# deeprob-org/deeprob-kit

Measured on AMD Instinct MI355X. Metric: log-likelihoods/sec, RAT-SPN D=784 batch=64k at 1/2/4/8 MI355X, higher is better.
Workload: dtype f32; 1 GPU; GaussianRatSpn(784, rg_depth=2, rg_repetitions=8, rg_batch=2, rg_sum=2) forward LL, 65536 samples per GPU per step, mean LL reduced on device; global_batch=65536, resident_batches=4

## Files before the change

### deeprob-kit_amd/csrc/ratspn_gemm_common.h

```cpp
#pragma once
#include "common.h"
#include <math.h>

namespace dpk {

typedef _Float16 half8 __attribute__((ext_vector_type(8)));
typedef _Float16 half4 __attribute__((ext_vector_type(4)));
typedef _Float16 half2 __attribute__((ext_vector_type(2)));
typedef float gf32x2 __attribute__((ext_vector_type(2)));
typedef float gf32x4 __attribute__((ext_vector_type(4)));
typedef float gf32x16 __attribute__((ext_vector_type(16)));

constexpr int kGemmWaves = 4;
constexpr int kGemmTile = 32 * kGemmWaves;
constexpr int kGemmStages = 3;
#ifndef DPK_X_NT
#define DPK_X_NT 0
#endif
constexpr bool kGemmXNonTemporal = DPK_X_NT != 0;
typedef __attribute__((address_space(3))) float lfloat;
typedef __attribute__((address_space(3))) unsigned lunsigned;
typedef __attribute__((address_space(3))) char lchar;
typedef const __attribute__((address_space(1))) char *gcchar_p;
typedef const __attribute__((address_space(1))) void *gvoid_p;
__host__ __device__ constexpr int gemm_ks(int NT) { return NT <= 2 ? 4 : 2; }
constexpr float kGemmStepBound = 1.0e6f;
constexpr float kGemmAbsBound = 1.0e3f;

__device__ __forceinline__ void split_f16(float v, _Float16 &hi, _Float16 &lo) {
    hi = (_Float16)v;
    lo = (_Float16)(v - (float)hi);
}

__device__ __forceinline__ void gemm_lds_barrier() {
    asm volatile("s_waitcnt lgkmcnt(0)\n\ts_barrier" ::: "memory");
}

template <bool NT = false>
__device__ __forceinline__ void glds16(unsigned voff, gcchar_p sbase_in, unsigned lds_dst_in) {
    const uint64_t sb = (uint64_t)(uintptr_t)sbase_in;
    const uint64_t sbase = ((uint64_t)(unsigned)__builtin_amdgcn_readfirstlane((int)(unsigned)(sb >> 32)) << 32) |
                           (uint64_t)(unsigned)__builtin_amdgcn_readfirstlane((int)(unsigned)sb);
    const unsigned lds_dst = (unsigned)__builtin_amdgcn_readfirstlane((int)lds_dst_in);
    unsigned keep;
    if constexpr (NT)
        asm volatile("s_mov_b32 %0, m0\n\ts_mov_b32 m0, %3\n\ts_nop 4\n\tglobal_load_lds_dwordx4 %1, %2 nt\n\ts_mov_b32 m0, %0"
                     : "=&s"(keep)
                     : "v"(voff), "s"(sbase), "s"(lds_dst)
                     : "memory");
    else
        asm volatile("s_mov_b32 %0, m0\n\ts_mov_b32 m0, %3\n\ts_nop 4\n\tglobal_load_lds_dwordx4 %1, %2\n\ts_mov_b32 m0, %0"
                     : "=&s"(keep)
                     : "v"(voff), "s"(sbase), "s"(lds_dst)
                     : "memory");
}

__device__ __forceinline__ void split8(const float (&v)[8], half8 &xh, half8 &xl) {
#ifdef DPK_SPLIT8_ASM
    typedef unsigned u32x4 __attribute__((ext_vector_type(4)));
    u32x4 hp, lp;
#pragma unroll
    for (int p = 0; p < 4; ++p) {
        unsigned h2, l2;
        float b0, b1;
        asm("v_cvt_pk_f16_f32 %0, %1, %2" : "=v"(h2) : "v"(v[2 * p]), "v"(v[2 * p + 1]));
        asm("v_cvt_f32_f16_e32 %0, %1" : "=v"(b0) : "v"(h2));
        asm("v_cvt_f32_f16_sdwa %0, %1 dst_sel:DWORD dst_unused:UNUSED_PAD src0_sel:WORD_1" : "=v"(b1) : "v"(h2));
        const float d0 = v[2 * p] - b0, d1 = v[2 * p + 1] - b1;
        asm("v_cvt_pk_f16_f32 %0, %1, %2" : "=v"(l2) : "v"(d0), "v"(d1));
        hp[p] = h2;
        lp[p] = l2;
    }
    xh = __builtin_bit_cast(half8, hp);
    xl = __builtin_bit_cast(half8, lp);
    return;
#endif
#pragma unroll
    for (int p = 0; p < 4; ++p) {
        const gf32x2 a = {v[2 * p], v[2 * p + 1]};
        const half2 h = __builtin_convertvector(a, half2);
        const gf32x2 b = __builtin_convertvector(h, gf32x2);
        const half2 l = __builtin_convertvector(a - b, half2);
        xh[2 * p] = h[0];
        xh[2 * p + 1] = h[1];
        xl[2 * p] = l[0];
        xl[2 * p + 1] = l[1];
    }
}


template <int KS, int PB, int PB2 = 0>
__device__ __forceinline__ void gemm_loader_run(const float *x, int64_t B, int D, int NCH, int ntiles, int tile0,
                                                int tstride, gcchar_p table, int chunk_table_bytes, int tab_kb0,
                                                unsigned smem_base, int stage_bytes, int wave, int lane,
                                                gcchar_p table2 = nullptr) {
    constexpr int KC = 16 * KS, W = 4 * KS, ROWB = KC * 4, RPI = 64 / W;
    constexpr int SWS = (W == 16) ? 0 : (W == 8 ? 1 : 2);
    constexpr int XB = kGemmTile * ROWB;
    constexpr int PX = 32 / RPI;
    constexpr int P = PX + PB + PB2;
    static_assert(P <= 63, "vmcnt field");
    unsigned voff[PX];
#pragma unroll
    for (int j = 0; j < PX; ++j) {
        const int rl = wave * 32 + j * RPI + lane / W;
        const int gp = (lane & (W - 1)) ^ ((rl >> SWS) & (W - 1));
        voff[j] = (unsigned)(rl * D + gp * 4) * 4u;
    }
    const unsigned toff = (unsigned)(tab_kb0 * 1024 + lane * 16);
    int ptile = tile0, pc = 0, pstage = 0;
    auto issue_next = [&]() {
        const int64_t b0 = (int64_t)ptile * kGemmTile;
        const gcchar_p xt = (gcchar_p)x + (b0 * D + pc * KC) * 4;
        const gcchar_p tsrc = table + (int64_t)pc * chunk_table_bytes;
        const unsigned st = smem_base + pstage * stage_bytes;
        const bool full = (b0 + kGemmTile <= B) && ((pc + 1) * KC <= D);
        if (full) {
#pragma unroll
            for (int j = 0; j < PX; ++j) glds16<kGemmXNonTemporal>(voff[j], xt, st + (wave * 32 + j * RPI) * ROWB);
        } else {
            const int nvalid = (int)min((int64_t)kGemmTile, B - b0);
            const int vp = min(W, (D - pc * KC) >> 2);
#pragma unroll
            for (int j = 0; j < PX; ++j) {
                const int rl = wave * 32 + j * RPI + lane / W;
                const int gp = min((lane & (W - 1)) ^ ((rl >> SWS) & (W - 1)), vp - 1);
                glds16<kGemmXNonTemporal>((unsigned)(min(rl, nvalid - 1) * D + gp * 4) * 4u, xt, st + (wave * 32 + j * RPI) * ROWB);
            }
        }
#pragma unroll
        for (int j = 0; j < PB; ++j) glds16(toff + j * 1024, tsrc, st + XB + tab_kb0 * 1024 + j * 1024);
        if constexpr (PB2 > 0) {
            const gcchar_p tsrc2 = table2 + (int64_t)pc * chunk_table_bytes;
#pragma unroll
            for (int j = 0; j < PB2; ++j)
                glds16((unsigned)((wave * PB2 + j) * 1024 + lane * 16), tsrc2, st + XB + chunk_table_bytes + (wave * PB2 + j) * 1024);
        }
        pstage = (pstage + 1 == kGemmStages) ? 0 : pstage + 1;
        if (++pc == NCH) {
            pc = 0;
            ptile += tstride;
        }
    };
    static_assert(kGemmStages == 3, "the counted waits leave exactly one chunk in flight");
#pragma unroll
    for (int g = 0; g < kGemmStages - 1; ++g)
        if (ptile < ntiles) issue_next();
    __syncthreads();
    for (int tile = tile0; tile < ntiles; tile += tstride) {
        for (int c = 0; c < NCH; ++c) {
            if (c + 1 < NCH || tile + tstride < ntiles) {
                asm volatile("s_waitcnt vmcnt(%0)" ::"n"(P) : "memory");
            } else {
                asm volatile("s_waitcnt vmcnt(0)" ::: "memory");
            }
            gemm_lds_barrier();
            if (ptile < ntiles) issue_next();
        }
    }
}

}
```

### deeprob-kit_amd/csrc/ratspn_gemm_slice.hip

```cpp
#include "ratspn_gemm_fused.h"
#include "ratspn_gemm_prep.h"
#include "../../include/deeprob_slice.h"
#include <stdlib.h>
#include <algorithm>
#include <atomic>
#include <mutex>
#include <type_traits>
#include <vector>

namespace dpk {

constexpr int kSliceCompute = 7;
constexpr int kSliceKW = 7;
constexpr int kSliceThreads = (kSliceCompute + 1) * 64;
constexpr int kSliceSlot = kSliceKW * 2048;

__host__ __device__ constexpr int slice_part_bytes(int NT) { return NT * 4 * 1024; }
__host__ __device__ constexpr int slice_lds_bytes(int NT, int w0_floats) {
    return kSliceCompute * kSliceSlot + kSliceCompute * slice_part_bytes(NT) + kSliceCompute * 256 + 128 + 1024 + 0 * w0_floats;
}

#ifdef DPK_TIMELINE
#define SL_STAMP(row, slot) do { __builtin_amdgcn_sched_barrier(0); if (a.dbg && lane == 0 && (row) < 16 && blockIdx.x < 256) a.dbg[(((int64_t)blockIdx.x * 8 + wave) * 16 + (row)) * 8 + (slot)] = __builtin_amdgcn_s_memtime(); __builtin_amdgcn_sched_barrier(0); } while (0)
#else
#define SL_STAMP(row, slot) do { } while (0)
#endif

template <int I, int S, int NT>
__device__ __forceinline__ void slice_exact_raw(const GemmArgs &a, const float *raw0, const float *rawr, int64_t bw0, int lane,
                                                LseScratch sc) {
    constexpr int RPT = 8 / I;
    constexpr int RH = (NT * RPT + 1) / 2;
    const int s = lane & 31, h = lane >> 5;
    const int64_t b = bw0 + s;
    const bool valid = b < a.B;
    const float *xr = a.x + (valid ? b : a.B - 1) * a.D;
    const int d = a.d;
    float n1[RH][2][S];
#pragma unroll
    for (int m = 0; m < RH; ++m) {
        const int rho = 2 * m + h;
        float leaf[4][I];
#pragma unroll
        for (int q = 0; q < 4; ++q)
#pragma unroll
            for (int k = 0; k < I; ++k) leaf[q][k] = 0.f;
        if (rho < a.reps) {
#pragma unroll
            for (int q = 0; q < 4; ++q) {
                const int r = rho * 4 + q;
                for (int j = 0; j < d; ++j) {
                    const int64_t o = (int64_t)r * d + j;
                    if (a.pad != nullptr && a.pad[o]) continue;
                    const float xv = xr[a.mask[o]];
#pragma unroll
                    for (int k = 0; k < I; ++k) {
                        const int64_t po = ((int64_t)r * I + k) * d + j;
                        const float mu = a.loc[po], sg = a.scale[po];
                        const float dlt = xv - mu;
                        leaf[q][k] += nan_to_num_f(fmaf(dlt * dlt, -0.5f / (sg * sg), -logf(sg) - kLogSqrt2Pi));
                    }
                }
            }
#pragma unroll
            for (int p = 0; p < 2; ++p)
                prodsum_node_raw<I, S>(leaf[2 * p], leaf[2 * p + 1], raw0 + ((int64_t)rho * 2 + p) * S * I * I, sc.slot, n1[m][p]);
        }
    }
    const int M = a.reps * S * S;
    double part = 0.0;
    for (int cl = 0; cl < a.C; ++cl) {
        const float lse_row = raw_row_lse(rawr + (int64_t)cl * M, M);
        float mm = -INFINITY, ss = 0.f;
#pragma unroll
        for (int m = 0; m < RH; ++m) {
            const int rho = 2 * m + h;
            if (rho < a.reps) {
                float pm, ps;
                root_partial_raw<S>(n1[m][0], n1[m][1], rawr + (int64_t)cl * M + rho * S * S, lse_row, sc.slot, pm, ps);
                lse_merge(mm, ss, pm, ps);
            }
        }
        const float om = __shfl_xor(mm, 32, 64), os = __shfl_xor(ss, 32, 64);
        lse_merge(mm, ss, om, os);
        const float ll = (mm > -INFINITY) ? mm + logf(ss) : -INFINITY;
        if (h == 0 && valid) {
            a.out[b * a.C + cl] = ll;
            part += (double)ll;
        }
    }
    if (a.ll_sum != nullptr) {
        part = wave_reduce_sum(part);
        if (lane == 0) atomicAdd(a.ll_sum, part);
    }
}

constexpr int kSliceShards = 16;
struct SliceVerify {
    unsigned long long verdict[kSliceShards];
    unsigned long long hashed, hashed_base;
    unsigned long long pad[14];
    struct { unsigned long long n, pad[15]; } tickets[kSliceShards];
};
static_assert(sizeof(SliceVerify) == kSliceVerifyBytes, "the workspace block behind the VerifyCtl (common.h)");
__device__ __forceinline__ SliceVerify *slice_verify_of(VerifyCtl *c) {
    return reinterpret_cast<SliceVerify *>(reinterpret_cast<char *>(c) + 64);
}
constexpr int kFpK = 32;
template <int K>
__device__ __forceinline__ void fpw_issue(const unsigned *p, int nwords, int tid, int nthreads, unsigned (&w)[K]) {
#pragma unroll
    for (int k = 0; k < K; ++k) {
        const int e = tid + nthreads * k;
        w[k] = p[e < nwords ? e : 0];
    }
}
template <int K>
__device__ __forceinline__ unsigned long long fpw_sum(const unsigned (&w)[K], int nwords, unsigned tag, int tid, int nthreads) {
    unsigned long long h = 0ull;
#pragma unroll
    for (int k = 0; k < K; ++k) {
        const int e = tid + nthreads * k;
        if (e < nwords) h += fp_word(w[k], (unsigned)e * 8u + tag);
    }
    return h;
}
typedef unsigned fp_u4 __attribute__((ext_vector_type(4)));
template <int K>
__device__ __forceinline__ void fpw_issue4(const unsigned *p, int nwords, int tid, int nthreads, fp_u4 (&w)[K]) {
    const fp_u4 *p4 = (const fp_u4 *)p;
#pragma unroll
    for (int k = 0; k < K; ++k) {
        const int e = tid + nthreads * k;
        w[k] = p4[4 * e < nwords ? e : 0];
    }
}
template <int K>
__device__ __forceinline__ unsigned long long fpw_sum4(const fp_u4 (&w)[K], int nwords, unsigned tag, int tid, int nthreads) {
    unsigned long long h = 0ull;
#pragma unroll
    for (int k = 0; k < K; ++k) {
        const int e = 4 * (tid + nthreads * k);
        if (e < nwords)
            h += (fp_word(w[k].x, (unsigned)e * 8u + tag) + fp_word(w[k].y, (unsigned)(e + 1) * 8u + tag)) +
                 (fp_word(w[k].z, (unsigned)(e + 2) * 8u + tag) + fp_word(w[k].w, (unsigned)(e + 3) * 8u + tag));
    }
    return h;
}
template <int I>
__device__ __forceinline__ unsigned long long slice_hash_share(const GemmPrepArgs &a, int blk, int tid, int nthreads) {
    constexpr int RPT = 8 / I;
    const int nrb = a.NT * RPT, d = a.d;
    if (blk < nrb) {
        if (blk >= a.reps) return 0ull;
        const int rho = blk;
        const int nm = 8 * d, npd = a.pad != nullptr ? d : 0, nl = 4 * I * d;
        const unsigned *pm = (const unsigned *)(a.mask + (int64_t)rho * 4 * d);
        const unsigned *pl = (const unsigned *)(a.loc + (int64_t)rho * 4 * I * d);
        const unsigned *ps = (const unsigned *)(a.scale + (int64_t)rho * 4 * I * d);
        const unsigned *pp = a.pad != nullptr ? (const unsigned *)(a.pad + (int64_t)rho * 4 * d) : pm;
        if (nl > kFpK * nthreads || nm > kFpK * nthreads || npd > 8 * nthreads || ((uintptr_t)pp & 3) != 0 ||
            (((uintptr_t)pm | (uintptr_t)pl | (uintptr_t)ps) & 15) != 0)
            return gemm_prep_hash_share<I>(a, blk, tid, nthreads);
        fp_u4 wm[kFpK / 4], wl[kFpK / 4], ws[kFpK / 4];
        unsigned wp[8];
        fpw_issue4(pm, nm, tid, nthreads, wm);
        fpw_issue4(pl, nl, tid, nthreads, wl);
        fpw_issue4(ps, nl, tid, nthreads, ws);
        fpw_issue(pp, npd > 0 ? npd : 1, tid, nthreads, wp);
        return (fpw_sum4(wm, nm, 1, tid, nthreads) + fpw_sum(wp, npd, 2, tid, nthreads)) +
               (fpw_sum4(wl, nl, 3, tid, nthreads) + fpw_sum4(ws, nl, 4, tid, nthreads));
    }
    constexpr int rpb = kGemmPrepThreads / 64;
    unsigned long long h = 0ull;
    unsigned wv[rpb];
    bool in[rpb];
    unsigned tg[rpb];
#pragma unroll
    for (int r = 0; r < rpb; ++r) {
        const int row = (blk - nrb) * rpb + r;
        int rr = row, m = -1;
#pragma unroll
        for (int mm = 0; mm < 3; ++mm) {
            if (m < 0) {
                if (rr < a.rows[mm]) m = mm;
                else rr -= a.rows[mm];
            }
        }
        const int n = m >= 0 ? a.n[m] : 0;
        if (n > nthreads) return gemm_prep_hash_share<I>(a, blk, tid, nthreads);
        in[r] = tid < n;
        const float *base = m >= 0 ? a.w[m] + (int64_t)rr * n : a.w[0];
        wv[r] = __float_as_uint(base[in[r] ? tid : 0]);
        tg[r] = (unsigned)tid * 8u + (5u + 8192u * (unsigned)row);
    }
#pragma unroll
    for (int r = 0; r < rpb; ++r)
        if (in[r]) h += fp_word(wv[r], tg[r]);
    return h;
}
template <int I>
__device__ __forceinline__ void slice_verify_share(const GemmPrepArgs &pa, int lane, lunsigned *ctl_l) {
    const int np = pa.np, G = (int)gridDim.x, g = (int)blockIdx.x;
    SliceVerify *sv = slice_verify_of(pa.ctl);
    const int shard = g & (kSliceShards - 1);
    if (g >= np) {
        if (lane == 0) {
            const unsigned long long t = __hip_atomic_fetch_add(&sv->tickets[shard].n, 1ull, __ATOMIC_RELAXED, __HIP_MEMORY_SCOPE_AGENT);
            ctl_l[0] = 0u;
            ctl_l[2] = (unsigned)t;
            ctl_l[3] = (unsigned)(t >> 32);
        }
        return;
    }
    const unsigned long long vold = __hip_atomic_load(&sv->verdict[lane & (kSliceShards - 1)], __ATOMIC_RELAXED, __HIP_MEMORY_SCOPE_AGENT);
    const unsigned long long hb = __hip_atomic_load(&sv->hashed_base, __ATOMIC_RELAXED, __HIP_MEMORY_SCOPE_AGENT);
    const unsigned long long stored = pa.hash[g];
    unsigned long long h = slice_hash_share<I>(pa, g, lane, 64);
#pragma unroll
    for (int o = 32; o > 0; o >>= 1) h += (unsigned long long)__shfl_xor((long long)h, o, 64);
    const bool mismatch = kPrepHashBase + (unsigned long long)g + h != stored;
    unsigned long long t = 0ull, r = 0ull;
    if (lane == 0) {
        t = __hip_atomic_fetch_add(&sv->tickets[shard].n, 1ull, __ATOMIC_RELAXED, __HIP_MEMORY_SCOPE_AGENT);
        r = __hip_atomic_fetch_add(&sv->hashed, 1ull + (mismatch ? (1ull << 32) : 0ull), __ATOMIC_RELAXED, __HIP_MEMORY_SCOPE_AGENT);
        ctl_l[0] = 0u;
        ctl_l[2] = (unsigned)t;
        ctl_l[3] = (unsigned)(t >> 32);
    }
    const unsigned rlo = (unsigned)__builtin_amdgcn_readfirstlane((int)(unsigned)r);
    const unsigned rhi = (unsigned)__builtin_amdgcn_readfirstlane((int)(unsigned)(r >> 32));
    const unsigned hblo = (unsigned)__builtin_amdgcn_readfirstlane((int)(unsigned)hb);
    const unsigned hbhi = (unsigned)__builtin_amdgcn_readfirstlane((int)(unsigned)(hb >> 32));
    if (rlo - hblo != (unsigned)(np - 1)) return;
    const unsigned mism_now = rhi + (mismatch ? 1u : 0u);
    const bool stale = mism_now != hbhi;
    if (lane == 0)
        __hip_atomic_store(&sv->hashed_base, ((unsigned long long)mism_now << 32) | (unsigned long long)(rlo + 1u), __ATOMIC_RELAXED,
                           __HIP_MEMORY_SCOPE_AGENT);
    if (lane < kSliceShards) {
        const int cnt = lane < G ? (G - 1 - lane) / kSliceShards + 1 : 0;
        __hip_atomic_store(&sv->verdict[lane], (((vold >> 1) + (unsigned long long)cnt) << 1) | (stale ? 1ull : 0ull), __ATOMIC_RELAXED,
                           __HIP_MEMORY_SCOPE_AGENT);
    }
    if (lane == 0) ctl_l[0] = 2u | (stale ? 1u : 0u);
}
__device__ __forceinline__ void slice_verdict_poll(const GemmPrepArgs &pa, lunsigned *ctl_l, unsigned long long until) {
    const int shard = (int)blockIdx.x & (kSliceShards - 1);
    const unsigned long long *vp = &slice_verify_of(pa.ctl)->verdict[shard];
    const unsigned long long n = ((unsigned long long)ctl_l[3] << 32) | ctl_l[2];
    while ((ctl_l[0] & 2u) == 0u && __builtin_amdgcn_s_memrealtime() < until) {
        const unsigned long long v = __hip_atomic_load(vp, __ATOMIC_RELAXED, __HIP_MEMORY_SCOPE_AGENT);
        if ((v >> 1) > n) ctl_l[0] = 2u | (unsigned)(v & 1ull);
        else __builtin_amdgcn_s_sleep(16);
    }
}
__device__ __forceinline__ void slice_verdict_wait(const GemmPrepArgs &pa, lunsigned *ctl_l) {
    if ((ctl_l[0] & 2u) != 0u) return;
    const int shard = (int)blockIdx.x & (kSliceShards - 1);
    const unsigned long long *vp = &slice_verify_of(pa.ctl)->verdict[shard];
    const unsigned long long n = ((unsigned long long)ctl_l[3] << 32) | ctl_l[2];
    unsigned long long v = __hip_atomic_load(vp, __ATOMIC_RELAXED, __HIP_MEMORY_SCOPE_AGENT);
    bool timed_out = false;
    if ((v >> 1) <= n) {
        const unsigned long long t0 = __builtin_amdgcn_s_memrealtime();
        do {
            __builtin_amdgcn_s_sleep(8);
            v = __hip_atomic_load(vp, __ATOMIC_RELAXED, __HIP_MEMORY_SCOPE_AGENT);
            timed_out = __builtin_amdgcn_s_memrealtime() - t0 > 100000000ull;
        } while ((v >> 1) <= n && !timed_out);
    }
    ctl_l[0] = 2u | ((v & 1ull) != 0ull || timed_out ? 1u : 0u);
}

template <int I, int S, int NT>
__global__ __launch_bounds__(kSliceThreads) void ratspn_gemm_slice_kernel(const GemmArgs a, const GemmPrepArgs pa) {
    constexpr int RPT = 8 / I;
    constexpr int NMAX = (I > S ? I : S);
    constexpr int KW = kSliceKW;
    constexpr int PW = slice_part_bytes(NT);
    constexpr float kL2E = 1.4426950408889634f, kLn2 = 0.6931471805599453f;
    static_assert(I == 2 && NT == 2 && NT * RPT == 8, "phase-2 roles: 8 repetitions x 2 partitions = the 16 lanes of a sample; one b128 per partition");
    typedef __attribute__((address_space(3))) const gf32x4 lf4;
    typedef __attribute__((address_space(3))) gf32x4 lf4w;

    extern __shared__ __attribute__((aligned(16))) char smem_generic[];
    lchar *smem = (lchar *)smem_generic;
    lchar *part_l = smem + kSliceCompute * kSliceSlot;
    lfloat *q_l = (lfloat *)(part_l + kSliceCompute * PW);
    lunsigned *flag_l = (lunsigned *)(q_l + kSliceCompute * 64);
    lunsigned *ctl_l = flag_l + 16;
    lfloat *c2_l = (lfloat *)(flag_l + 32);

    const int tid = threadIdx.x;
    const int lane = tid & 63;
    const int wave = __builtin_amdgcn_readfirstlane(tid >> 6);
    const int s = lane & 31, h = lane >> 5;
    const int D = a.D;
    const int nblk = a.ntiles;
    const int first = (int)blockIdx.x, stride = (int)gridDim.x;
    const bool slicer = wave < kSliceCompute;
    SL_STAMP(15, 0);
    unsigned long long t_poll = 0ull;
    if (!slicer && pa.np > 0) {
        const unsigned long long t_entry = __builtin_amdgcn_s_memrealtime();
        __builtin_amdgcn_s_setprio(3);
        slice_verify_share<I>(pa, lane, ctl_l);
        __builtin_amdgcn_s_setprio(0);
        t_poll = t_entry + (a.ntiles > (int)gridDim.x ? 500ull : 450ull);
    }

    const int k0 = wave * KW;
    lchar *my = smem + (slicer ? wave : 0) * kSliceSlot;
    const unsigned my_u = (unsigned)(uintptr_t)my;
    unsigned voff[2];
#pragma unroll
    for (int i = 0; i < 2; ++i) {
        const int P = i * 64 + lane, drow = P >> 2, dcol = (P & 3) ^ ((drow >> 2) & 3);
        voff[i] = (unsigned)(drow * D + k0 * 16 + dcol * 4) * 4u;
    }
    auto issue_kk = [&](gcchar_p xt, int nvalid, int kk) {
        if (nvalid >= 32) {
            glds16<kGemmXNonTemporal>(voff[0] + kk * 64u, xt, my_u + kk * 2048);
            glds16<kGemmXNonTemporal>(voff[1] + kk * 64u, xt, my_u + kk * 2048 + 1024);
        } else {
#pragma unroll
            for (int i = 0; i < 2; ++i) {
                const int P = i * 64 + lane, drow = P >> 2, dcol = (P & 3) ^ ((drow >> 2) & 3);
                glds16<kGemmXNonTemporal>((unsigned)(min(drow, nvalid - 1) * D + (k0 + kk) * 16 + dcol * 4) * 4u, xt,
                                          my_u + kk * 2048 + i * 1024);
            }
        }
    };
    auto issue = [&](int blk) {
        const int64_t b0 = (int64_t)blk * 32;
        const gcchar_p xt = (gcchar_p)(a.x + b0 * D);
        const int nvalid = (int)min((int64_t)32, a.B - b0);
#pragma unroll
        for (int kk = 0; kk < KW; ++kk) issue_kk(xt, nvalid, kk);
    };
    const int nit = first < nblk ? (nblk - first + stride - 1) / stride : 0;
    lchar *tl = part_l + (slicer ? wave : 0) * PW;
    static_assert(PW >= KW * NT * kSliceTabBytes + 1024, "compact table + keep-masks in the wave's partial block");
    if (slicer && nit > 0) {
        const unsigned tl_u = (unsigned)(uintptr_t)tl;
        glds16<false>((unsigned)lane * 16u, (gcchar_p)pa.smask + wave * 1024, tl_u + KW * NT * kSliceTabBytes);
#pragma unroll
        for (int kk = 0; kk < KW; ++kk)
            glds16<false>((unsigned)lane * 16u, (gcchar_p)pa.stab + (int64_t)(k0 + kk) * NT * kSliceTabBytes,
                          tl_u + kk * NT * kSliceTabBytes);
        issue(first);
    }
    half8 mh[KW][NT], ml[KW][NT];
    typedef unsigned gu32x4 __attribute__((ext_vector_type(4)));
    typedef __attribute__((address_space(3))) const gu32x4 lu4;
    typedef __attribute__((address_space(3))) const unsigned short lushort;
#define DPK_SL_TABLE_EXPAND(kk)                                                                                                \
    do {                                                                                                                      \
        const unsigned bits = *(lushort *)(tl + KW * NT * kSliceTabBytes + lane * 16 + (kk) * 2);                             \
        const lchar *te = tl + (kk) * NT * kSliceTabBytes + ((lane >> 5) * 8 + ((lane >> 3) & 3) * 2 + (lane & 1)) * 16;      \
        _Pragma("unroll") for (int t = 0; t < NT; ++t) {                                                                      \
            gu32x4 hi = *(lu4 *)(te + t * kSliceTabBytes);                                                                    \
            gu32x4 lo = *(lu4 *)(te + t * kSliceTabBytes + kSliceTabBytes / 2);                                               \
            _Pragma("unroll") for (int jj = 0; jj < 4; ++jj) {                                                                \
                const int e0 = __builtin_amdgcn_sbfe((int)bits, t * 8 + 2 * jj, 1);                                           \
                const int e1 = __builtin_amdgcn_sbfe((int)bits, t * 8 + 2 * jj + 1, 1);                                       \
                const unsigned keep = ((unsigned)e0 & 0xFFFFu) | ((unsigned)e1 & 0xFFFF0000u);                                \
                hi[jj] &= keep;                                                                                               \
                lo[jj] &= keep;                                                                                               \
            }                                                                                                                 \
            mh[kk][t] = __builtin_bit_cast(half8, hi);                                                                        \
            ml[kk][t] = __builtin_bit_cast(half8, lo);                                                                        \
        }                                                                                                                     \
    } while (0)
    const int sl = lane >> 4, j = lane & 15;
    const int rho = j >> 1, p = j & 1;
    const int s2 = wave * 4 + sl;
    const bool active = rho < a.reps;
    const int rc = active ? rho : a.reps - 1;
    const int t2 = rc / RPT, ap = rc - t2 * RPT;
    static_assert(S * I * I == 8 && 2 * I == 4 && S * S == 4, "slot record layout");
    if (wave == 7 && sl == 0) {
        const float *wp = a.W0 + ((int64_t)(rc * 2 + p) * S) * I * I;
#pragma unroll
        for (int e = 0; e < S * I * I; ++e) c2_l[j * 16 + e] = wp[e];
#pragma unroll
        for (int qq = 0; qq < 2; ++qq)
#pragma unroll
            for (int k = 0; k < I; ++k) c2_l[j * 16 + 8 + qq * I + k] = a.biasT[(p * NT + t2) * 16 + (ap * 2 + qq) * I + k];
#pragma unroll
        for (int e = 0; e < S * S; ++e) c2_l[j * 16 + 12 + e] = ((const float *)a.Wr)[rc * S * S + e];
    }
    if (!slicer && pa.np > 0 && lane == 0) slice_verdict_poll(pa, ctl_l, t_poll);
    bool model_ok;
    {
        cint_p ce = as_const(a.elig);
        unsigned bits = 0u;
#pragma unroll
        for (int e = 0; e < NT * RPT; ++e) bits |= (ce[e] != 0 ? 1u : 0u) << e;
        model_ok = ((bits >> rc) & 1u) != 0u;
    }
    const int M = a.reps * S * S;
    const float *wr0 = (const float *)a.Wr + rc * S * S;
    if (tid < 16) flag_l[tid] = 0u;

    const int sw = (s >> 2) & 3;
    constexpr int XROW = 64, XKK = 2048;
    const lchar *xr0 = my + s * XROW + (((h * 2) ^ sw) << 4);
    const lchar *xr1 = my + s * XROW + (((h * 2 + 1) ^ sw) << 4);
    lchar *pw = part_l + (slicer ? wave : 0) * PW + s * 256;

    double ll_part = 0.0, pend_part = 0.0;
    bool saw_nan = false;
    unsigned long long exact_mask = 0ull;
    gf32x16 acc[NT];
    float qlane = 0.f;
#define DPK_SL_KSTEP(kk, v, tq2)                                                                                              \
    do {                                                                                                                      \
        _Pragma("unroll") for (int i = 0; i < 8; i += 2) {                                                                    \
            const gf32x2 pv = {v[i], v[i + 1]};                                                                               \
            tq2 = __builtin_elementwise_fma(pv, pv, tq2);                                                                     \
        }                                                                                                                     \
        half8 xh, xl;                                                                                                         \
        split8(v, xh, xl);                                                                                                    \
        _Pragma("unroll") for (int t = 0; t < NT; ++t) acc[t] = __builtin_amdgcn_mfma_f32_32x32x16_f16(mh[kk][t], xh, acc[t], 0, 0, 0); \
        _Pragma("unroll") for (int t = 0; t < NT; ++t) acc[t] = __builtin_amdgcn_mfma_f32_32x32x16_f16(mh[kk][t], xl, acc[t], 0, 0, 0); \
        _Pragma("unroll") for (int t = 0; t < NT; ++t) acc[t] = __builtin_amdgcn_mfma_f32_32x32x16_f16(ml[kk][t], xh, acc[t], 0, 0, 0); \
    } while (0)
    if (slicer && nit > 0) {
        const bool more = nit > 1;
        const int64_t nb0 = (int64_t)(first + stride) * 32;
        const gcchar_p nxt = (gcchar_p)(a.x + nb0 * D);
        const int nnv = (int)min((int64_t)32, a.B - nb0);
#pragma unroll
        for (int t = 0; t < NT; ++t)
#pragma unroll
            for (int i = 0; i < 16; ++i) acc[t][i] = 0.f;
        gf32x2 tq2 = {0.f, 0.f};
        gf32x4 xa0, xa1, xb0, xb1;
        asm volatile("s_waitcnt vmcnt(14)" ::: "memory");
        DPK_SL_TABLE_EXPAND(0);
        asm volatile("s_waitcnt vmcnt(12)" ::: "memory");
        xa0 = *(lf4 *)(xr0);
        xa1 = *(lf4 *)(xr1);
#define DPK_SL_FIRST_STEP(kk, NW_MORE, NW_LAST)                                                                               \
    do {                                                                                                                      \
        asm volatile("s_waitcnt lgkmcnt(0)" ::: "memory");                                                                    \
        if (more && (kk) <= 2) issue_kk(nxt, nnv, kk);                                                                        \
        float v[8];                                                                                                           \
        _Pragma("unroll") for (int i = 0; i < 4; ++i) {                                                                       \
            v[i] = xa0[i];                                                                                                    \
            v[4 + i] = xa1[i];                                                                                                \
        }                                                                                                                     \
        if ((kk) + 1 < KW) {                                                                                                  \
            if (more) asm volatile("s_waitcnt vmcnt(%0)" ::"n"(NW_MORE) : "memory");                                          \
            else asm volatile("s_waitcnt vmcnt(%0)" ::"n"(NW_LAST) : "memory");                                               \
            xb0 = *(lf4 *)(xr0 + ((kk) + 1) * XKK);                                                                           \
            xb1 = *(lf4 *)(xr1 + ((kk) + 1) * XKK);                                                                           \
        }                                                                                                                     \
        if ((kk) + 1 < KW) DPK_SL_TABLE_EXPAND(((kk) + 1 < KW ? (kk) + 1 : 0));                                               \
        DPK_SL_KSTEP(kk, v, tq2);                                                                                             \
        xa0 = xb0;                                                                                                            \
        xa1 = xb1;                                                                                                            \
    } while (0)
        DPK_SL_FIRST_STEP(0, 12, 10);
        DPK_SL_FIRST_STEP(1, 12, 8);
        DPK_SL_FIRST_STEP(2, 12, 6);
        DPK_SL_FIRST_STEP(3, 10, 4);
        DPK_SL_FIRST_STEP(4, 8, 2);
        DPK_SL_FIRST_STEP(5, 6, 0);
        DPK_SL_FIRST_STEP(6, 0, 0);
#undef DPK_SL_FIRST_STEP
#undef DPK_SL_TABLE_EXPAND
        qlane = tq2[0] + tq2[1];
        if (more) {
            issue_kk(nxt, nnv, 3);
            issue_kk(nxt, nnv, 4);
        }
    }
    SL_STAMP(15, 1);
    [[maybe_unused]] int row = 0;
    int it = 0;
    for (; it < nit; ++it) {
        const int blk = first + it * stride;
        const bool more = it + 1 < nit;
        const bool more2 = it + 2 < nit;
        SL_STAMP(row, 0);
        gemm_lds_barrier();
        SL_STAMP(row, 1);
        if (slicer) {
#pragma unroll
            for (int t = 0; t < NT; ++t)
#pragma unroll
                for (int i4 = 0; i4 < 4; ++i4) {
                    const int g = t * 4 + i4;
                    const gf32x4 o = {acc[t][4 * i4], acc[t][4 * i4 + 1], acc[t][4 * i4 + 2], acc[t][4 * i4 + 3]};
                    *(lf4w *)(pw + (((g * 2 + h) ^ (s & 7)) << 4)) = o;
                }
            q_l[wave * 64 + lane] = qlane;
        }
        if (it > 0) {
            const lunsigned *fl = flag_l + ((it - 1) & 1) * 8;
            const unsigned any_bad = (unsigned)__builtin_amdgcn_readfirstlane(
                (int)((fl[0] | fl[1]) | (fl[2] | fl[3]) | (fl[4] | fl[5]) | (fl[6] | fl[7])));
            if (any_bad) exact_mask |= 1ull << (it - 1);
            else ll_part += pend_part;
        }
        gemm_lds_barrier();
        if (slicer && more) {
            const int64_t nb0 = (int64_t)(first + (it + 1) * stride) * 32;
            const gcchar_p nxt = (gcchar_p)(a.x + nb0 * D);
            const int nnv = (int)min((int64_t)32, a.B - nb0);
            issue_kk(nxt, nnv, 5);
            issue_kk(nxt, nnv, 6);
        }
        SL_STAMP(row, 2);

        int jo = j;
        asm volatile("" : "+v"(jo));
        const lchar *pr = part_l + s2 * 256 + ((jo ^ (s2 & 7)) << 4);
        const lfloat *qr = q_l + (jo < 2 * kSliceCompute ? (jo >> 1) * 64 + (jo & 1) * 32 + s2 : 0);
        gf32x4 lf = *(lf4 *)pr;
#pragma unroll
        for (int w = 1; w < kSliceCompute; ++w) lf += *(lf4 *)(pr + w * PW);
        float qv = *qr;
        qv = j < 2 * kSliceCompute ? qv : 0.f;
        const float qtot = row16_sum(qv);
        const int64_t b2 = (int64_t)blk * 32 + s2;
        saw_nan = saw_nan || (qtot != qtot);
        bool bad = !(qtot <= kExpandBound * kExpandBound * (float)D) || (active && !model_ok);
        const lf4 *c2 = (const lf4 *)(c2_l + jo * 16);
        const gf32x4 w0a = c2[0], w0b = c2[1], cs4 = c2[2], wr4 = c2[3];
        const float w0[S][I * I] = {{w0a[0], w0a[1], w0a[2], w0a[3]}, {w0b[0], w0b[1], w0b[2], w0b[3]}};
        float va[I], vc[I];
#pragma unroll
        for (int k = 0; k < I; ++k) {
            va[k] = lf[k] + cs4[k];
            vc[k] = lf[I + k] + cs4[I + k];
        }
        float ea[I], ec[I];
        const float ma = exp2_children<I>(va, ea), mc = exp2_children<I>(vc, ec);
        float n1[S];
#pragma unroll
        for (int o = 0; o < S; ++o) {
            float v = 0.f;
#pragma unroll
            for (int i = 0; i < I; ++i) {
                float tt = 0.f;
#pragma unroll
                for (int jj = 0; jj < I; ++jj) tt = fmaf(w0[o][i * I + jj], ec[jj], tt);
                v = fmaf(ea[i], tt, v);
            }
            n1[o] = fmaf(__builtin_amdgcn_logf(v), kLn2, ma + mc);
            bad = bad || (v < 1e-30f && active);
        }
        float ta[S], tc[S];
#pragma unroll
        for (int o = 0; o < S; ++o) {
            const float other = dpp_f<kDppXor1>(n1[o]);
            ta[o] = p == 0 ? n1[o] : other;
            tc[o] = p == 0 ? other : n1[o];
        }
        float ra[S], rcx[S];
        const float m2 = exp2_children<S>(ta, ra) + exp2_children<S>(tc, rcx);
        const float mr = active ? m2 : -INFINITY;
        const float mtop = row16_max(mr);
        const float mtop0 = (mtop == -INFINITY) ? 0.f : mtop;
        const float scale = (active && p == 0) ? __builtin_amdgcn_exp2f((mr - mtop0) * kL2E) : 0.f;
        const float qterm = -0.5f * qtot;
        const bool writer = j == 0 && b2 < a.B;
        double part = 0.0;
        for (int cl = 0; cl < a.C; ++cl) {
            float wr[S * S];
            if (cl == 0) {
#pragma unroll
                for (int e = 0; e < S * S; ++e) wr[e] = wr4[e];
            } else {
#pragma unroll
                for (int e = 0; e < S * S; ++e) wr[e] = wr0[(int64_t)cl * M + e];
            }
            float v = 0.f;
#pragma unroll
            for (int i = 0; i < S; ++i) {
                float tt = 0.f;
#pragma unroll
                for (int jj = 0; jj < S; ++jj) tt = fmaf(wr[i * S + jj], rcx[jj], tt);
                v = fmaf(ra[i], tt, v);
            }
            bad = bad || (v < 1e-30f && mr > -INFINITY);
            const float tot = row16_sum(v * scale);
            const float ll = ((mtop > -INFINITY) ? fmaf(__builtin_amdgcn_logf(tot), kLn2, mtop) : -INFINITY) + qterm;
            if (writer) {
                a.out[b2 * a.C + cl] = ll;
                part += (double)ll;
            }
        }
        pend_part = part;
        const bool wave_bad = __any(bad);
        if (lane == 0) flag_l[(it & 1) * 8 + wave] = wave_bad ? 1u : 0u;
        SL_STAMP(row, 3);
        if (slicer && more) {
            const int64_t nb2 = (int64_t)(first + (it + 2) * stride) * 32;
            const gcchar_p nxt = (gcchar_p)(a.x + nb2 * D);
            const int nnv = (int)min((int64_t)32, a.B - nb2);
#pragma unroll
            for (int t = 0; t < NT; ++t)
#pragma unroll
                for (int i = 0; i < 16; ++i) acc[t][i] = 0.f;
            gf32x2 tq2 = {0.f, 0.f};
            gf32x4 xa0, xa1, xb0, xb1;
#define DPK_SL_LAND(p)                                                                                                        \
    do {                                                                                                                      \
        if (more2) asm volatile("s_waitcnt vmcnt(%0)" ::"n"(2 * (6 - (p)) + 2 * ((p) < 3 ? (p) : 3)) : "memory");              \
        else asm volatile("s_waitcnt vmcnt(%0)" ::"n"(12 - 2 * (p)) : "memory");                                              \
    } while (0)
            DPK_SL_LAND(0);
            xa0 = *(lf4 *)(xr0);
            xa1 = *(lf4 *)(xr1);
#define DPK_SL_STEP(kk)                                                                                                       \
    do {                                                                                                                      \
                                     \
        asm volatile("s_waitcnt lgkmcnt(0)" ::: "memory");                                                                    \
        if (more2 && (kk) <= 2) issue_kk(nxt, nnv, kk);                                                                       \
        float v[8];                                                                                                           \
        _Pragma("unroll") for (int i = 0; i < 4; ++i) {                                                                       \
            v[i] = xa0[i];                                                                                                    \
            v[4 + i] = xa1[i];                                                                                                \
        }                                                                                                                     \
        if ((kk) + 1 < KW) {                                                                                                  \
            DPK_SL_LAND(((kk) + 1 < KW ? (kk) + 1 : 6));                                                                      \
            xb0 = *(lf4 *)(xr0 + ((kk) + 1) * XKK);                                                                           \
            xb1 = *(lf4 *)(xr1 + ((kk) + 1) * XKK);                                                                           \
        }                                                                                                                     \
        DPK_SL_KSTEP(kk, v, tq2);                                                                                             \
        xa0 = xb0;                                                                                                            \
        xa1 = xb1;                                                                                                            \
    } while (0)
            DPK_SL_STEP(0);
            DPK_SL_STEP(1);
            DPK_SL_STEP(2);
            DPK_SL_STEP(3);
            DPK_SL_STEP(4);
            DPK_SL_STEP(5);
            DPK_SL_STEP(6);
#undef DPK_SL_STEP
#undef DPK_SL_LAND
            qlane = tq2[0] + tq2[1];
            if (more2) {
                issue_kk(nxt, nnv, 3);
                issue_kk(nxt, nnv, 4);
            }
        }
        SL_STAMP(row, 4);
        ++row;
    }
    SL_STAMP(15, 2);
    if (pa.np > 0 && !slicer && lane == 0) slice_verdict_wait(pa, ctl_l);
    __syncthreads();
    const bool tables_stale = pa.np > 0 && (ctl_l[0] & 1u) != 0u;
    if (it > 0) {
        const lunsigned *fl = flag_l + ((it - 1) & 1) * 8;
        const unsigned any_bad = (fl[0] | fl[1]) | (fl[2] | fl[3]) | (fl[4] | fl[5]) | (fl[6] | fl[7]);
        if (any_bad) exact_mask |= 1ull << (it - 1);
        else ll_part += pend_part;
    }
    if (tables_stale) {
        ll_part = 0.0;
        exact_mask = nit >= 64 ? ~0ull : ((1ull << nit) - 1ull);
    }
    if (a.ll_sum != nullptr) {
        double *red_l = reinterpret_cast<double *>(smem_generic + kSliceCompute * kSliceSlot);
        double red = ll_part + __shfl_xor(ll_part, 16, 64);
        red += __shfl_xor(red, 32, 64);
        if (lane == 0) red_l[wave] = red;
        __syncthreads();
        if (tid == 0) {
            double tot = 0.0;
#pragma unroll
            for (int w = 0; w < 8; ++w) tot += red_l[w];
            atomicAdd(a.ll_sum + (a.ll_cnt > 1 ? ((int)blockIdx.x & 15) : 0), tot);
            if (blockIdx.x == 0) atomicAdd(a.ll_sum + a.ll_cnt, (double)a.B * (double)a.C);
        }
    }
    if (__any(saw_nan) && lane == 0 && a.slow_flag != nullptr) *a.slow_flag = a.launch_seq;
    if (exact_mask != 0ull) {
        int tid_x = (int)threadIdx.x;
        asm volatile("" : "+v"(tid_x));
        const int lane_x = tid_x & 63;
        LseScratch sc{reinterpret_cast<float *>(smem_generic) + tid_x * (2 * NMAX)};
        int n = 0;
        for (int e = 0; e < 64; ++e) {
            if (!((exact_mask >> e) & 1ull)) continue;
            if ((n++ & 7) != wave) continue;
            if (tables_stale) slice_exact_raw<I, S, NT>(a, pa.w[0], pa.w[1], (int64_t)(first + e * stride) * 32, lane_x, sc);
            else gemm_exact_body<I, S, NT>(a, (int64_t)(first + e * stride) * 32, lane_x, sc);
        }
    }
    if (tables_stale && (int)blockIdx.x < pa.np) {
        __syncthreads();
        gemm_prep_block<I>(pa, (int)blockIdx.x, reinterpret_cast<int *>(smem_generic), kPrepBuild);
    }
}

bool gemm_slice_shape_ok(int D, int reps, int I, int S, int NT) {
    if (!(I == 2 && S == 2) || NT != 2) return false;
    if (D != 16 * kSliceCompute * kSliceKW) return false;
    return slice_lds_bytes(NT, reps * 2 * S * I * I) <= 160 * 1024;
}

constexpr int64_t kSliceBatchDefault = 7681;
static int64_t slice_batch_initial() {
    const char *e = getenv("DPK_GEMM_SLICE_MIN");
    return e ? (int64_t)atoll(e) : kSliceBatchDefault;
}
static int64_t &slice_batch_min_ref() {
    static int64_t v = slice_batch_initial();
    return v;
}
int64_t gemm_slice_min_batch() { return slice_batch_min_ref(); }

static int slice_gmax(int64_t ntiles, int cus, int lanes, int np) {
    const int share = std::max(1, cus / std::max(1, lanes));
    return (int)std::max<int64_t>(share, std::min<int64_t>(np, ntiles));
}
int slice_grid(int64_t ntiles, int cus, int lanes, int np) {
    if (ntiles <= 0 || cus <= 0) return 0;
    if (lanes <= 1) return (int)std::min<int64_t>(ntiles, cus);
    const int gmax = slice_gmax(ntiles, cus, lanes, np);
    const int64_t rounds = cdiv(ntiles, (int64_t)gmax);
    const int64_t grid = cdiv(ntiles, rounds);
    return (int)std::max<int64_t>(grid, std::min<int64_t>(np, ntiles));
}

constexpr int kSliceLanesMax = DPS_LANES_MAX;
constexpr int kSliceAutoLanesMax = DPS_AUTO_LANES_MAX;
constexpr int kSliceAutoStreak = DPS_AUTO_STREAK;
constexpr int kSliceAutoRecheck = DPS_AUTO_RECHECK;
constexpr int kSlicePeers = 8;
constexpr int kSliceDevices = 64;
static int slice_lanes_initial() {
    const char *e = getenv("DPK_SLICE_LANES");
    const int v = e ? atoi(e) : 0;
    return v < 0 ? 0 : std::min(v, kSliceLanesMax);
}
static std::atomic<int> &slice_lanes_ref() {
    static std::atomic<int> v{slice_lanes_initial()};
    return v;
}
static std::atomic<int> g_slice_last_grid{0}, g_slice_last_lanes{0};

namespace {
struct SlicePeer {
    const void *ws;
    hipStream_t st;
    int streak;
    int lanes;
    int since;
    unsigned long long seq;
};
struct SliceRegistry {
    std::mutex mu;
    std::vector<SlicePeer> dev[kSliceDevices];
    unsigned long long seq = 0;
};
SliceRegistry &slice_registry() {
    static SliceRegistry r;
    return r;
}
}

void slice_lanes_forget(const void *lo, const void *hi) {
    SliceRegistry &r = slice_registry();
    std::lock_guard<std::mutex> lock(r.mu);
    for (auto &v : r.dev)
        v.erase(std::remove_if(v.begin(), v.end(), [&](const SlicePeer &e) { return (const char *)e.ws >= (const char *)lo && (const char *)e.ws < (const char *)hi; }),
                v.end());
}

static int slice_lanes_auto(const void *ws_key, hipStream_t st) {
    int d = 0;
    if (hipGetDevice(&d) != hipSuccess || d < 0 || d >= kSliceDevices) {
        (void)hipGetLastError();
        return 1;
    }
    SliceRegistry &r = slice_registry();
    std::lock_guard<std::mutex> lock(r.mu);
    std::vector<SlicePeer> &v = r.dev[d];
    for (SlicePeer &e : v)
        if (e.ws == ws_key && e.st == st && e.lanes > 1 && e.since + 1 < kSliceAutoRecheck) {
            ++e.since;
            e.seq = ++r.seq;
            return e.lanes;
        }
    int busy = 0;
    for (size_t i = 0; i < v.size();) {
        bool gone = false;
        if (v[i].ws != ws_key && v[i].st != st) {
            hipStreamCaptureStatus cs = hipStreamCaptureStatusNone;
            hipError_t e = hipStreamIsCapturing(v[i].st, &cs);
            if (e == hipSuccess && cs == hipStreamCaptureStatusNone) e = hipStreamQuery(v[i].st);
            if (e == hipErrorNotReady) ++busy;
            if (e != hipSuccess) (void)hipGetLastError();
            gone = e != hipSuccess && e != hipErrorNotReady;
        }
        if (gone) {
            v[i] = v.back();
            v.pop_back();
        } else {
            ++i;
        }
    }
    size_t me = 0;
    while (me < v.size() && v[me].ws != ws_key) ++me;
    if (me >= v.size()) {
        if ((int)v.size() >= kSlicePeers) {
            size_t old = 0;
            for (size_t i = 1; i < v.size(); ++i)
                if (v[i].seq < v[old].seq) old = i;
            v[old] = v.back();
            v.pop_back();
        }
        v.push_back(SlicePeer{ws_key, st, 0, 1, 0, 0ull});
        me = v.size() - 1;
    }
    SlicePeer &m = v[me];
    m.st = st;
    m.seq = ++r.seq;
    m.streak = busy > 0 ? std::min(m.streak + 1, kSliceAutoStreak) : 0;
    m.lanes = m.streak >= kSliceAutoStreak ? std::min(1 + busy, kSliceAutoLanesMax) : 1;
    m.since = 0;
    return m.lanes;
}

int gemm_slice_lanes(const void *ws_key, uint32_t flags, hipStream_t st) {
    const int forced = slice_lanes_ref().load(std::memory_order_relaxed);
    if (forced >= 1) return forced;
    const int stated = (int)((flags & DPK_FLAG_SLICE_LANES_MASK) >> DPK_FLAG_SLICE_LANES_SHIFT);
    if (stated >= 1) return stated;
    hipStreamCaptureStatus cs = hipStreamCaptureStatusNone;
    if (hipStreamIsCapturing(st, &cs) != hipSuccess) {
        (void)hipGetLastError();
        return 1;
    }
    if (cs != hipStreamCaptureStatusNone) return 1;
    return slice_lanes_auto(ws_key, st);
}

template <int I, int S, int NT>
static int gemm_slice_launch(const GemmArgs &a0, const GemmPrepArgs &p, int lanes, hipStream_t st) {
    size_t lds = (size_t)slice_lds_bytes(NT, a0.reps * 2 * S * I * I);
    if (p.np > 0 && gemm_prep_lds_bytes(a0.D, I, a0.d) > lds) lds = gemm_prep_lds_bytes(a0.D, I, a0.d);
    DPK_REQUIRE(lds <= 160 * 1024, DPK_EUNSUPPORTED, "ratspn_gemm_slice: %zu bytes of LDS", lds);
    auto kern = ratspn_gemm_slice_kernel<I, S, NT>;
    if (int rc = ensure_dynamic_lds(reinterpret_cast<const void *>(kern), 160 * 1024)) return rc;
    const int cus = device_cus();
    Profile prof(DPK_KERNEL_RATSPN_FUSED, st);
    const int64_t per_launch = (int64_t)64 * 32 * slice_gmax(cdiv(a0.B, 32), cus, lanes, p.np);
    for (int64_t off = 0; off < a0.B; off += per_launch) {
        GemmArgs a = a0;
        a.x = a0.x + off * a0.D;
        a.out = a0.out + off * a0.C;
        a.B = std::min(per_launch, a0.B - off);
        a.ntiles = cdiv(a.B, 32);
        const int grid = slice_grid(a.ntiles, cus, lanes, p.np);
        DPK_REQUIRE(grid >= 1 && grid >= std::min<int64_t>(p.np, a.ntiles) && cdiv((int64_t)a.ntiles, (int64_t)grid) <= 64, DPK_ELAUNCH,
                    "ratspn_gemm_slice: grid %d for %lld blocks", grid, (long long)a.ntiles);
        GemmPrepArgs pp = p;
        pp.readers = grid;
#ifdef DPK_TIMELINE
        a.dbg = timeline_buffer("_slice", (size_t)256 * 8 * 16 * 8 * 8, grid);
#endif
        DPK_LAUNCH("ratspn_gemm_slice_kernel", kern, dim3(grid), dim3(kSliceThreads), lds, st, a, pp);
        g_slice_last_grid.store(grid, std::memory_order_relaxed);
        g_slice_last_lanes.store(lanes, std::memory_order_relaxed);
    }
    prof.stop();
    return DPK_OK;
}

bool gemm_slice_checks_inline(int64_t B, int np, int d, int lanes) {
    const int cus = device_cus();
    const int64_t ntiles = cdiv(B, 32);
    return B <= (int64_t)64 * 32 * slice_gmax(ntiles, cus, lanes, np) && ntiles >= np &&
           slice_grid(ntiles, cus, lanes, np) >= np && 8 * d <= kFpK * 64;
}

int ratspn_gemm_slice_forward(const GemmArgs &a, const GemmPrepArgs &p, int I, int S, int NT, int lanes, hipStream_t st) {
    if (I == 2 && S == 2 && NT == 2) return gemm_slice_launch<2, 2, 2>(a, p, std::max(1, lanes), st);
    set_error("ratspn_gemm_slice: (channels=%d, sums=%d) not built", I, S);
    return DPK_EUNSUPPORTED;
}

}

extern "C" int64_t dpk_ratspn_slice_batch_min(int64_t samples) {
    int64_t &v = dpk::slice_batch_min_ref();
    const int64_t prev = v;
    v = samples < -1 ? dpk::slice_batch_initial() : samples;
    return prev;
}

extern "C" int32_t dps_slice_grid(int64_t ntiles, int32_t cus, int32_t lanes, int32_t np) {
    return dpk::slice_grid(ntiles, cus, lanes, np);
}
extern "C" int32_t dps_slice_lanes(int32_t lanes) {
    std::atomic<int> &v = dpk::slice_lanes_ref();
    const int next = lanes < 0 ? dpk::slice_lanes_initial() : std::min<int>(lanes, dpk::kSliceLanesMax);
    return v.exchange(next, std::memory_order_relaxed);
}
extern "C" int32_t dps_slice_last_grid(void) { return dpk::g_slice_last_grid.load(std::memory_order_relaxed); }
extern "C" int32_t dps_slice_last_lanes(void) { return dpk::g_slice_last_lanes.load(std::memory_order_relaxed); }
```

### include/deeprob_slice.h

```cpp
#ifndef DEEPROB_SLICE_H
#define DEEPROB_SLICE_H

#include <stdint.h>

#ifdef __cplusplus
extern "C" {
#endif

#define DPS_LANES_MAX 15
#define DPS_AUTO_LANES_MAX 4
#define DPS_AUTO_STREAK 4
#define DPS_AUTO_RECHECK 8

int32_t dps_slice_grid(int64_t ntiles, int32_t cus, int32_t lanes, int32_t np);

int32_t dps_slice_lanes(int32_t lanes);

int32_t dps_slice_last_grid(void);
int32_t dps_slice_last_lanes(void);

#ifdef __cplusplus
}
#endif
#endif
```

Measured before the change: 1.674 billion log-likelihoods/sec.

## Use fma_mix for fp16 split residual and add slice-lane reentry hysteresis

Replaces the f16 hi/lo split's convert-back-and-subtract with v_fma_mix_f32, which computes the residual straight from the packed f16 high part. This removes a conversion per element in the GEMM inner loop. Separately, the auto slice-lane heuristic gains a resume/gap state so it can go back to multi-lane slicing right after a brief idle gap instead of rebuilding the busy streak. The two changes are unrelated: one is inline asm in the hot loop, the other is host-side scheduling hysteresis.

```diff
diff --git a/deeprob-kit_amd/csrc/ratspn_gemm_common.h b/deeprob-kit_amd/csrc/ratspn_gemm_common.h
--- a/deeprob-kit_amd/csrc/ratspn_gemm_common.h
+++ b/deeprob-kit_amd/csrc/ratspn_gemm_common.h
@@ -88,6 +88,25 @@
     }
 }
 
+__device__ __forceinline__ void split8_mix(const float (&v)[8], half8 &xh, half8 &xl) {
+#pragma unroll
+    for (int p = 0; p < 4; ++p) {
+        const gf32x2 a = {v[2 * p], v[2 * p + 1]};
+        const half2 h = __builtin_convertvector(a, half2);
+        const unsigned hb = __builtin_bit_cast(unsigned, h);
+        gf32x2 d;
+        float d0, d1;
+        asm("v_fma_mix_f32 %0, %1, -1.0, %2 op_sel:[0,0,0] op_sel_hi:[1,0,0]" : "=v"(d0) : "v"(hb), "v"(a[0]));
+        asm("v_fma_mix_f32 %0, %1, -1.0, %2 op_sel:[1,0,0] op_sel_hi:[1,0,0]" : "=v"(d1) : "v"(hb), "v"(a[1]));
+        d[0] = d0;
+        d[1] = d1;
+        const half2 l = __builtin_convertvector(d, half2);
+        xh[2 * p] = h[0];
+        xh[2 * p + 1] = h[1];
+        xl[2 * p] = l[0];
+        xl[2 * p + 1] = l[1];
+    }
+}
 
 template <int KS, int PB, int PB2 = 0>
 __device__ __forceinline__ void gemm_loader_run(const float *x, int64_t B, int D, int NCH, int ntiles, int tile0,
diff --git a/deeprob-kit_amd/csrc/ratspn_gemm_slice.hip b/deeprob-kit_amd/csrc/ratspn_gemm_slice.hip
--- a/deeprob-kit_amd/csrc/ratspn_gemm_slice.hip
+++ b/deeprob-kit_amd/csrc/ratspn_gemm_slice.hip
@@ -1,5 +1,6 @@
 #include "ratspn_gemm_fused.h"
 #include "ratspn_gemm_prep.h"
+#include "ratspn_slice_lanes.h"
 #include "../../include/deeprob_slice.h"
 #include <stdlib.h>
 #include <algorithm>
@@ -422,7 +423,7 @@
             tq2 = __builtin_elementwise_fma(pv, pv, tq2);                                                                     \
         }                                                                                                                     \
         half8 xh, xl;                                                                                                         \
-        split8(v, xh, xl);                                                                                                    \
+        split8_mix(v, xh, xl);                                                                                                \
         _Pragma("unroll") for (int t = 0; t < NT; ++t) acc[t] = __builtin_amdgcn_mfma_f32_32x32x16_f16(mh[kk][t], xh, acc[t], 0, 0, 0); \
         _Pragma("unroll") for (int t = 0; t < NT; ++t) acc[t] = __builtin_amdgcn_mfma_f32_32x32x16_f16(mh[kk][t], xl, acc[t], 0, 0, 0); \
         _Pragma("unroll") for (int t = 0; t < NT; ++t) acc[t] = __builtin_amdgcn_mfma_f32_32x32x16_f16(ml[kk][t], xh, acc[t], 0, 0, 0); \
@@ -736,6 +737,7 @@
 constexpr int kSliceAutoLanesMax = DPS_AUTO_LANES_MAX;
 constexpr int kSliceAutoStreak = DPS_AUTO_STREAK;
 constexpr int kSliceAutoRecheck = DPS_AUTO_RECHECK;
+constexpr int kSliceAutoReentry = DPS_AUTO_REENTRY;
 constexpr int kSlicePeers = 8;
 constexpr int kSliceDevices = 64;
 static int slice_lanes_initial() {
@@ -747,14 +749,20 @@
     static std::atomic<int> v{slice_lanes_initial()};
     return v;
 }
+static int slice_reentry() {
+    static const int v = [] {
+        const char *e = getenv("DPK_SLICE_REENTRY");
+        return e ? std::max(0, atoi(e)) : kSliceAutoReentry;
+    }();
+    return v;
+}
 static std::atomic<int> g_slice_last_grid{0}, g_slice_last_lanes{0};
 
 namespace {
 struct SlicePeer {
     const void *ws;
     hipStream_t st;
-    int streak;
-    int lanes;
+    SliceLaneState look;
     int since;
     unsigned long long seq;
 };
@@ -787,10 +795,10 @@
     std::lock_guard<std::mutex> lock(r.mu);
     std::vector<SlicePeer> &v = r.dev[d];
     for (SlicePeer &e : v)
-        if (e.ws == ws_key && e.st == st && e.lanes > 1 && e.since + 1 < kSliceAutoRecheck) {
+        if (e.ws == ws_key && e.st == st && e.look.lanes > 1 && e.since + 1 < kSliceAutoRecheck) {
             ++e.since;
             e.seq = ++r.seq;
-            return e.lanes;
+            return e.look.lanes;
         }
     int busy = 0;
     for (size_t i = 0; i < v.size();) {
@@ -820,16 +828,15 @@
             v[old] = v.back();
             v.pop_back();
         }
-        v.push_back(SlicePeer{ws_key, st, 0, 1, 0, 0ull});
+        v.push_back(SlicePeer{ws_key, st, SliceLaneState{0, 1, 0, 0}, 0, 0ull});
         me = v.size() - 1;
     }
     SlicePeer &m = v[me];
     m.st = st;
     m.seq = ++r.seq;
-    m.streak = busy > 0 ? std::min(m.streak + 1, kSliceAutoStreak) : 0;
-    m.lanes = m.streak >= kSliceAutoStreak ? std::min(1 + busy, kSliceAutoLanesMax) : 1;
+    m.look = slice_lanes_next(m.look, busy, kSliceAutoStreak, kSliceAutoLanesMax, slice_reentry());
     m.since = 0;
-    return m.lanes;
+    return m.look.lanes;
 }
 
 int gemm_slice_lanes(const void *ws_key, uint32_t flags, hipStream_t st) {
diff --git a/deeprob-kit_amd/csrc/ratspn_slice_lanes.h b/deeprob-kit_amd/csrc/ratspn_slice_lanes.h
--- /dev/null
+++ b/deeprob-kit_amd/csrc/ratspn_slice_lanes.h
@@ -0,0 +1,39 @@
+#pragma once
+
+namespace dpk {
+
+struct SliceLaneState {
+    int streak;
+    int lanes;
+    int resume;
+    int gap;
+};
+
+inline SliceLaneState slice_lanes_next(SliceLaneState s, int busy, int streak_min, int lanes_max, int reentry) {
+    if (busy > 0) {
+        s.streak = s.streak + 1 < streak_min ? s.streak + 1 : streak_min;
+        if (s.streak >= streak_min) {
+            s.lanes = 1 + busy < lanes_max ? 1 + busy : lanes_max;
+        } else if (s.resume > 1 && s.gap < reentry) {
+            s.lanes = s.resume;
+            s.streak = streak_min;
+        } else {
+            s.lanes = 1;
+        }
+        s.resume = 0;
+        s.gap = 0;
+        return s;
+    }
+    if (s.lanes > 1) {
+        s.resume = s.lanes;
+        s.gap = 0;
+    } else if (s.resume > 1 && ++s.gap >= reentry) {
+        s.resume = 0;
+        s.gap = 0;
+    }
+    s.streak = 0;
+    s.lanes = 1;
+    return s;
+}
+
+}
diff --git a/include/deeprob_slice.h b/include/deeprob_slice.h
--- a/include/deeprob_slice.h
+++ b/include/deeprob_slice.h
@@ -11,6 +11,7 @@
 #define DPS_AUTO_LANES_MAX 4
 #define DPS_AUTO_STREAK 4
 #define DPS_AUTO_RECHECK 8
+#define DPS_AUTO_REENTRY 8
 
 int32_t dps_slice_grid(int64_t ntiles, int32_t cus, int32_t lanes, int32_t np);
 
```

Result: faster. 1.694 billion log-likelihoods/sec (median of 6 runs) (+1.2%).
